# warmshao/ChatTTSPlus

Hardware: AMD Instinct MI355X
Metric: decode tokens/s (higher is better)
Workload: dtype f32

## Files before the change

### chatttsplus_amd/csrc/persist_layer.hip

```cpp
#include "kernels.h"
#include "persist.h"

typedef unsigned long long u64;

#ifndef PL_LB
#define PL_LB PL_THREADS_MAX
#endif
#define PL_SPIN_LIMIT (1u << 18)

typedef __attribute__((address_space(3))) int pl_lds_int;
#define PL_ABORT_GET(p_) __hip_atomic_load((pl_lds_int*)(p_), __ATOMIC_RELAXED, __HIP_MEMORY_SCOPE_WORKGROUP)
#define PL_ABORT_SET(p_) __hip_atomic_store((pl_lds_int*)(p_), 1, __ATOMIC_RELAXED, __HIP_MEMORY_SCOPE_WORKGROUP)
__device__ inline void store_granule(u64* g, unsigned tag, float v) {
    __hip_atomic_store(g, ((u64)tag << 32) | (u64)__builtin_bit_cast(unsigned, v), __ATOMIC_RELAXED, __HIP_MEMORY_SCOPE_AGENT);
}

template <int N, typename OffFn>
__device__ inline bool sweep(const u64* base, unsigned lane_elem, OffFn off, unsigned tag, float (&v)[N], int* err, int code, int* abort_s, int nap = 1) {
    const u64* p = base + lane_elem;
    asm volatile("" : "+v"(p));
#pragma unroll 1
    for (unsigned spins = 0;; ++spins) {
        bool ok = true;
#pragma unroll
// ... 705 lines not shown
                }
                if (last) PL_MARK(3);
                for (int z = 0; z < a.delay_att; ++z) __builtin_amdgcn_s_sleep(2);
                {
                    if (EW == 2 && (a.poll & 1)) watch_sentinels(a.g_att, [ew](int i) { return (i / 6) * PL_H + 64 * (2 * (i % 6) + ew) + 63; }, 6 * R, tag, lane, abort_s);
                    float v[GX * R];
                    const bool got = PL_SWEEP(GX * R, a.g_att, PL_G_ATT, (unsigned)e, [](int k) { return (k / GX) * PL_H + NE * (k % GX); }, tag, v, 3);
                    (void)got;
#pragma unroll
                    for (int k = 0; k < GX * R; ++k) xs[(k / GX) * PL_H + NE * (k % GX) + e] = v[k];
                }
                if (last) PL_MARK(4);
                PL_B1();
                float ldo = 0.f;
                float uo[LORA ? 16 : 1];
                const int slO = (LORA && e < 4 * R) ? pl_slot(a.lslots, e >> 2) : -1;
                if constexpr (LORA) {
                    for (int z = 0; z < a.delay_u; ++z) __builtin_amdgcn_s_sleep(2);
                    const bool got = sweep_masked<16>(a.g_u, (unsigned)((e >> 2) * 64 + 48), slO >= 0, tag, uo, a.error, 10, abort_s, a.nap);
                    (void)got;
                }
                __syncthreads();
                if constexpr (LORA) {
                    if (slO >= 0) {
                        const float* const bo = lbs + 192 * R + (e >> 2) * 64 + (e & 3) * 16;
#pragma unroll
                        for (int k = 0; k < 16; ++k) ldo = fmaf(bo[k], uo[k], ldo);
                    }
                }
                if (e < 4 * R) {
                    const int i = e & 3, r = e >> 2;
                    const float x1 = xres[4 * r + i] + (pl_red(red, i, r) + ldo);
                    xres[4 * r + i] = x1;
                    if (!(a.fault > 0 && b == 5 && l + 1 == a.fault))
                        store_granule(a.g_x1 + (size_t)pl_opq<(R > PL_MAXR_ONE)>(r * PL_H + 4 * b + i), tag, x1);
                }
                if (last) PL_MARK(5);
                for (int z = 0; z < a.delay; ++z) __builtin_amdgcn_s_sleep(2);
                {
                    if (EW == 2 && (a.poll & 1)) watch_sentinels(a.g_x1, [ew](int i) { return (R - 1) * PL_H + 4 * (16 * (2 * (i >> 4) + ew) + (i & 15)) + 3; }, 96, tag, lane, abort_s);
                    float v[GX * R];
                    const bool got = PL_SWEEP(GX * R, a.g_x1, PL_G_X1, (unsigned)e, [](int k) { return (k / GX) * PL_H + NE * (k % GX); }, tag, v, 4);
                    (void)got;
#pragma unroll
                    for (int r = 0; r < R; ++r) ssp[r] = 0.f;
#pragma unroll
                    for (int k = 0; k < GX * R; ++k) {
                        xs[(k / GX) * PL_H + NE * (k % GX) + e] = v[k];
                        ssp[k / GX] += v[k] * v[k];
                    }
#pragma unroll
                    for (int r = 0; r < R; ++r) {
                        const float s = wave_sum(ssp[r]);
                        if (lane == 0) ssq[ew * R + r] = s;
                    }
                }
                if (last) PL_MARK(6);
                PL_B1();
                __syncthreads();
                if constexpr (A16) {
                    float av = 0.f;
                    const int pi = e & 15, r = e >> 4;
                    if (e < 16 * R) {
                        const int w = pi >> 1, p = pi & 1;
                        const float rs = 1.0f / sqrtf((EW == 2 ? ssq[r] + ssq[R + r] : (ssq[r] + ssq[R + r]) + (ssq[2 * R + r] + ssq[3 * R + r])) / (float)PL_H + a.eps);
                        const float gv = pl_red(red, w, 16 * p + r) * rs, uv = pl_red(red, w, 16 * p + R + r) * rs;
                        av = (gv / (1.0f + expf(-gv))) * uv;
                    }
                    const float a1 = __shfl_down(av, 1), a2 = __shfl_down(av, 2);
                    if (e < 16 * R && pi % 3 == 0)
                        store_granule16(a.g_act, PL_GEMV_BLOCKS * PL_A16_SLOTS * R, (unsigned)pl_opq<(R > PL_MAXR_ONE)>((r * PL_GEMV_BLOCKS + b) * PL_A16_SLOTS + pi / 3), tag,
                                        av, (pi + 1 < 16) ? a1 : 0.f, (pi + 2 < 16) ? a2 : 0.f);
                } else if (e < 16 * R) {
                    const int pi = e & 15, r = e >> 4, w = pi >> 1, p = pi & 1;
                    const float rs = 1.0f / sqrtf((EW == 2 ? ssq[r] + ssq[R + r] : (ssq[r] + ssq[R + r]) + (ssq[2 * R + r] + ssq[3 * R + r])) / (float)PL_H + a.eps);
                    const float gv = pl_red(red, w, 16 * p + r) * rs, uv = pl_red(red, w, 16 * p + R + r) * rs;
                    store_granule(a.g_act + (size_t)pl_opq<(R > PL_MAXR_ONE)>(r * PL_I + 16 * b + pi), tag, (gv / (1.0f + expf(-gv))) * uv);
                }
                if (last) PL_MARK(7);
                for (int z = 0; z < a.delay_act; ++z) __builtin_amdgcn_s_sleep(2);
                if constexpr (A16) {
                    constexpr int TOT = PL_GEMV_BLOCKS * PL_A16_SLOTS * R, NK = (TOT + NE - 1) / NE;
                    constexpr int NC = (NK + PL_A16_CHUNK - 1) / PL_A16_CHUNK, CH = (NK + NC - 1) / NC;
                    act16_chunk<0, (NK < CH ? NK : CH), NE, TOT>(a.g_act, e, tag, (__attribute__((address_space(3))) float*)xs, a.error, abort_s, a.nap);
                    if constexpr (NC > 1) act16_chunk<CH, (NK - CH < CH ? NK - CH : CH), NE, TOT>(a.g_act, e, tag, (__attribute__((address_space(3))) float*)xs, a.error, abort_s, a.nap);
                    if constexpr (NC > 2) act16_chunk<2 * CH, (NK - 2 * CH < CH ? NK - 2 * CH : CH), NE, TOT>(a.g_act, e, tag, (__attribute__((address_space(3))) float*)xs, a.error, abort_s, a.nap);
                    if constexpr (NC > 3) act16_chunk<3 * CH, (NK - 3 * CH < CH ? NK - 3 * CH : CH), NE, TOT>(a.g_act, e, tag, (__attribute__((address_space(3))) float*)xs, a.error, abort_s, a.nap);
                    if constexpr (NC > 4) act16_chunk<4 * CH, NK - 4 * CH, NE, TOT>(a.g_act, e, tag, (__attribute__((address_space(3))) float*)xs, a.error, abort_s, a.nap);
                    static_assert(NC <= 5, "act gather: more chunks");
                } else {
                if (EW == 2 && (a.poll & 1)) watch_sentinels(a.g_act, [ew](int i) { return (R - 1) * PL_I + 16 * (8 * (i >> 2) + 4 * ew + (i & 3)) + 15; }, 96, tag, lane, abort_s);
                if constexpr (EW == 2) {
#pragma unroll
                    for (int r = 0; r < R; ++r) {
                        float v[24];
                        const bool got = sweep<24>(a.g_act, (unsigned)(r * PL_I + e), [](int k) { return 128 * k; }, tag, v, a.error, 5, abort_s, a.nap);
                        (void)got;
#pragma unroll
                        for (int k = 0; k < 24; ++k) xs[r * PL_I + 128 * k + e] = v[k];
                    }
                } else {
#ifdef PL_EXP_E1
                    if constexpr (R > PL_MAXR_ONE) {
#pragma unroll
                        for (int r = 0; r < R; ++r) {
                            float v[12];
                            const bool got = PL_SWEEP(12, a.g_act, PL_G_ACT, (unsigned)(r * PL_I + e), [](int k) { return 256 * k; }, tag, v, 5);
                            (void)got;
#pragma unroll
                            for (int k = 0; k < 12; ++k) xs[r * PL_I + 256 * k + e] = v[k];
                        }
                    } else
#endif
#pragma unroll
                    for (int r = 0; r + 1 < R; r += 2) {
                        float v[24];
                        const bool got = PL_SWEEP(24, a.g_act, PL_G_ACT, (unsigned)(r * PL_I + e), [](int k) { return (k / 12) * PL_I + 256 * (k % 12); }, tag, v, 5);
                        (void)got;
#pragma unroll
                        for (int k = 0; k < 24; ++k) xs[(r + k / 12) * PL_I + 256 * (k % 12) + e] = v[k];
                    }
#ifdef PL_EXP_E1
                    if constexpr ((R & 1) != 0 && R <= PL_MAXR_ONE) {
#else
                    if constexpr ((R & 1) != 0) {
#endif
                        constexpr int r = R - 1;
                        float v[12];
                        const bool got = PL_SWEEP(12, a.g_act, PL_G_ACT, (unsigned)(r * PL_I + e), [](int k) { return 256 * k; }, tag, v, 5);
                        (void)got;
#pragma unroll
                        for (int k = 0; k < 12; ++k) xs[r * PL_I + 256 * k + e] = v[k];
                    }
                }
                }
                if (last) PL_MARK(8);
                PL_B1();
                __syncthreads();
                if (e < 4 * R) {
                    const int i = e & 3, r = e >> 2;
                    const float x2 = xres[4 * r + i] + (pl_red(red, 2 * i, r) + pl_red(red, 2 * i + 1, r));
                    if (last && !a.heads) a.x[(size_t)r * PL_H + 4 * b + i] = x2;
                    else {
                        xres[4 * r + i] = x2;
                        store_granule(a.g_x + (size_t)pl_opq<(R > PL_MAXR_ONE)>(r * PL_H + 4 * b + i), tag, x2);
                    }
                }
            }
            if (a.heads) {
                const unsigned tagh = tag0 + (unsigned)(NL - 1);
                int4 hst = make_int4(1, 0, 0, 0);
                int hout = 0;
                float lnf_v = 0.f;
                if (e < 4 * R) {
                    hst = *(const int4*)(a.rows + (e >> 2));
                    hout = a.rows[e >> 2].out;
                    lnf_v = a.lnf[4 * b + (e & 3)];
                }
                for (int z = 0; z < a.delay_x; ++z) __builtin_amdgcn_s_sleep(2);
                float v[GX * R];
                const bool got = PL_SWEEP(GX * R, a.g_x, PL_G_X, (unsigned)e, [](int k) { return (k / GX) * PL_H + NE * (k % GX); }, tagh, v, 1);
                (void)got;
#pragma unroll
                for (int r = 0; r < R; ++r) ssp[r] = 0.f;
#pragma unroll
                for (int k = 0; k < GX * R; ++k) {
                    xs[(k / GX) * PL_H + NE * (k % GX) + e] = v[k];
                    ssp[k / GX] += v[k] * v[k];
                }
#pragma unroll
                for (int r = 0; r < R; ++r) {
                    const float s = wave_sum(ssp[r]);
                    if (lane == 0) ssq[ew * R + r] = s;
                }
                PL_B1();
                __syncthreads();
                if (e < PL_HEAD_ROWS * R) {
                    const int rr = e % PL_HEAD_ROWS, r = e / PL_HEAD_ROWS, col = PL_HEAD_ROWS * b + rr;
                    const float rs = 1.0f / sqrtf((EW == 2 ? ssq[r] + ssq[R + r] : (ssq[r] + ssq[R + r]) + (ssq[2 * R + r] + ssq[3 * R + r])) / (float)PL_H + a.eps);
                    if (col < a.n_valid) a.logits[(size_t)r * a.n_valid + col] = pl_red(red, rr >> 1, (rr & 1) * R + r) * rs;
                }
                if (e < 4 * R) {
                    float* const hid_out = ((SamplerDynPtr)a.dyn)->hidden_out;
                    if (hid_out != nullptr && hst.x == 0) {
                        const int i = e & 3, r = e >> 2;
                        const float rs = 1.0f / sqrtf((EW == 2 ? ssq[r] + ssq[R + r] : (ssq[r] + ssq[R + r]) + (ssq[2 * R + r] + ssq[3 * R + r])) / (float)PL_H + a.eps);
                        hid_out[(size_t)hout * ((SamplerDynPtr)a.dyn)->hidden_stride + (size_t)hst.y * PL_H + 4 * b + i] = lnf_v * (xres[4 * r + i] * rs);
                    }
                }
            }
            PL_MARK(9);
            if (a.ts != nullptr && e == 0) {
#pragma unroll
                for (int i = 0; i < 10; ++i) a.ts[(size_t)b * 10 + i] = t_mark[i];
            }
            if (b == 0 && e == 0) __hip_atomic_fetch_add(a.epoch, 1u, __ATOMIC_RELAXED, __HIP_MEMORY_SCOPE_AGENT);
        }
        return;
    }

    constexpr bool PAIR = R > PL_MAXR_ONE;
    constexpr int NWI = PAIR ? 4 : 8;
    const int S = PAIR ? 1 : a.S;
    const int isub = PAIR ? ((wave < 8) ? (wave >> 2) : ((wave - 8) & 1)) : 0;
    const int iw = PAIR ? (wave & 3) : wave;
    const int item = PAIR ? 2 * (b - PL_GEMV_BLOCKS) + isub : b - PL_GEMV_BLOCKS;
    if ((PAIR ? 2 * (b - PL_GEMV_BLOCKS) : item) >= PL_NH * R * S) return;
    const int rh = item / S, sp = item - rh * S;
    const int r = rh / PL_NH, hh = rh % PL_NH;
    float* const qs = att_s + 64 * isub;
    float* const ks = att_s + 128 + 64 * isub;
    float* const vs = att_s + 256 + 64 * isub;
    float* const mo = att_s + 384;
    float* const mm = mo + 512;
    float* const ml = mm + 8;
    const size_t kv_per = a.kv_per;
    if (wave < 8) {
        const RowMeta m = a.meta[r];
        const int kvc = (m.slot - m.kv_start + S - 1) / S;
        const int kv0 = m.kv_start + sp * kvc, kv1 = min(kv0 + kvc, m.slot);
        const int grp = lane >> 3, sub = lane & 7;
        const size_t head_base = ((size_t)m.seq * PL_NH + hh) * a.Lmax * CTTS_HEAD_DIM;
        constexpr int PRE = 6;
        constexpr int NT = (PAIR || PL_TAIL_ALL) ? PL_TAIL_IT : 0, PT = PRE + NT;
        constexpr int TB = sizeof(WT) == 4 ? 4096 : 2048;
        typedef __attribute__((address_space(3))) char lds_c;
        typedef __attribute__((address_space(1))) const void* gptr_t;
        lds_c* const tl = (lds_c*)smem + PL_FRONT_BYTES + wave * (NT * TB);
        PlKV<WT> kf[PRE];
        typename KvElem<WT>::reg vv[PRE][8];
        bool ok[PT];
        bool any_ok[PT];
#pragma unroll
        for (int u = 0; u < PT; ++u) {
            const int p = kv0 + 8 * (iw + NWI * u) + grp;
            ok[u] = p < kv1;
            any_ok[u] = kv0 + 8 * (iw + NWI * u) < kv1;
        }
#define PL_LOAD_KV(l_) do { const WT* const kb_ = (const WT*)a.kv + (size_t)(l_) * 2 * kv_per + head_base; const WT* const vb_ = kb_ + kv_per + lane; \
        _Pragma("unroll") for (int u = 0; u < PRE; ++u) if (any_ok[u]) { const int p0_ = kv0 + 8 * (iw + NWI * u); const int pc_ = ok[u] ? p0_ + grp : m.kv_start; \
            kf[u].load(kb_ + (size_t)pc_ * CTTS_HEAD_DIM + 8 * sub); \
            _Pragma("unroll") for (int g = 0; g < 8; ++g) vv[u][g] = KvElem<WT>::load(vb_ + (size_t)min(p0_ + g, kv1 - 1) * CTTS_HEAD_DIM); } } while (0)
#define PL_DMA_KV(l_) do { if constexpr (NT > 0) { const WT* const kb_ = (const WT*)a.kv + (size_t)(l_) * 2 * kv_per + head_base; const WT* const vb_ = kb_ + kv_per; \
        int ln_ = lane; asm volatile("" : "+v"(ln_));       \
        const int grp = ln_ >> 3, sub = ln_ & 7, lane = ln_; \
        _Pragma("unroll") for (int t = 0; t < NT; ++t) if (any_ok[PRE + t]) { const int p0_ = kv0 + 8 * (iw + NWI * (PRE + t)); \
            const WT* const ks_ = kb_ + (size_t)min(p0_ + grp, kv1 - 1) * CTTS_HEAD_DIM + 8 * sub; \
            if constexpr (sizeof(WT) == 4) { \
                __builtin_amdgcn_global_load_lds((gptr_t)ks_, (__attribute__((address_space(3))) void*)(tl + t * TB), 16, 0, 0); \
                __builtin_amdgcn_global_load_lds((gptr_t)(ks_ + 4), (__attribute__((address_space(3))) void*)(tl + t * TB + 1024), 16, 0, 0); \
                const WT* const v0_ = vb_ + (size_t)min(p0_ + (lane >> 4), kv1 - 1) * CTTS_HEAD_DIM + 4 * (lane & 15); \
                const WT* const v1_ = vb_ + (size_t)min(p0_ + 4 + (lane >> 4), kv1 - 1) * CTTS_HEAD_DIM + 4 * (lane & 15); \
                __builtin_amdgcn_global_load_lds((gptr_t)v0_, (__attribute__((address_space(3))) void*)(tl + t * TB + 2048), 16, 0, 0); \
                __builtin_amdgcn_global_load_lds((gptr_t)v1_, (__attribute__((address_space(3))) void*)(tl + t * TB + 3072), 16, 0, 0); \
            } else { \
                __builtin_amdgcn_global_load_lds((gptr_t)ks_, (__attribute__((address_space(3))) void*)(tl + t * TB), 16, 0, 0); \
                const WT* const v0_ = vb_ + (size_t)min(p0_ + grp, kv1 - 1) * CTTS_HEAD_DIM + 8 * sub; \
                __builtin_amdgcn_global_load_lds((gptr_t)v0_, (__attribute__((address_space(3))) void*)(tl + t * TB + 1024), 16, 0, 0); \
            } } } } while (0)
        PL_DMA_KV(0);
        PL_LOAD_KV(0);
        __builtin_amdgcn_sched_barrier(0);
        if (__builtin_amdgcn_readfirstlane(done_v | err_v)) return;
        __syncthreads();
        for (int l = 0; l < NL; ++l) {
            const WT* const kb = (const WT*)a.kv + (size_t)l * 2 * kv_per + head_base + 8 * sub;
            const WT* const vb = (const WT*)a.kv + (size_t)l * 2 * kv_per + kv_per + head_base + lane;
            __syncthreads();
#define PL_AMARK(i) do { if (a.ts != nullptr && l + 1 == NL && tid == 0) a.ts[(size_t)b * 10 + (i)] = wall_clock64(); } while (0)
            PL_AMARK(3);
            const f32x4 q0 = *(const f32x4*)(qs + 8 * sub), q1 = *(const f32x4*)(qs + 8 * sub + 4);
            float sc[PT];
            float mw = -INFINITY;
#pragma unroll
            for (int u = 0; u < PRE; ++u) {
                sc[u] = -INFINITY;
                if (any_ok[u]) {
                    float dot = q0[0] * kf[u].at(0) + q0[1] * kf[u].at(1) + q0[2] * kf[u].at(2) + q0[3] * kf[u].at(3) +
                                q1[0] * kf[u].at(4) + q1[1] * kf[u].at(5) + q1[2] * kf[u].at(6) + q1[3] * kf[u].at(7);
                    dot += dpp_f<DPP_XOR1>(dot);
                    dot += dpp_f<DPP_XOR2>(dot);
                    dot += dpp_f<DPP_HALF_MIRROR>(dot);
                    sc[u] = ok[u] ? dot : -INFINITY;
                    mw = fmaxf(mw, sc[u]);
                }
            }
            if constexpr (NT > 0) {
                asm volatile("s_waitcnt vmcnt(0)" ::: "memory");
#pragma unroll
                for (int t = 0; t < NT; ++t) {
                    sc[PRE + t] = -INFINITY;
                    if (any_ok[PRE + t]) {
                        PlKV<WT> kt;
                        if constexpr (sizeof(WT) == 4) { kt.a = *(const __attribute__((address_space(3))) f32x4*)(tl + t * TB + lane * 16); kt.b = *(const __attribute__((address_space(3))) f32x4*)(tl + t * TB + 1024 + lane * 16); }
                        else kt.h = *(const __attribute__((address_space(3))) half8*)(tl + t * TB + lane * 16);
                        float dot = q0[0] * kt.at(0) + q0[1] * kt.at(1) + q0[2] * kt.at(2) + q0[3] * kt.at(3) + q1[0] * kt.at(4) + q1[1] * kt.at(5) + q1[2] * kt.at(6) + q1[3] * kt.at(7);
                        dot += dpp_f<DPP_XOR1>(dot);
                        dot += dpp_f<DPP_XOR2>(dot);
                        dot += dpp_f<DPP_HALF_MIRROR>(dot);
                        sc[PRE + t] = ok[PRE + t] ? dot : -INFINITY;
                        mw = fmaxf(mw, sc[PRE + t]);
                    }
                }
            }
            float mrun = wave_max(mw);
            PL_AMARK(4);
            float lrun = 0.f;
            float oa[4] = {0.f, 0.f, 0.f, 0.f};
#pragma unroll
            for (int u = 0; u < PRE; ++u) {
                if (any_ok[u]) {
                    const float pe = (sc[u] == -INFINITY) ? 0.f : expf(sc[u] - mrun);
                    lrun += pe;
#pragma unroll
                    for (int g = 0; g < 8; ++g) oa[g & 3] = fmaf(readlane_f(pe, 8 * g), KvElem<WT>::f(vv[u][g]), oa[g & 3]);
                }
            }
            if constexpr (NT > 0) {
#pragma unroll
                for (int t = 0; t < NT; ++t) {
                    if (any_ok[PRE + t]) {
                        const float pe = (sc[PRE + t] == -INFINITY) ? 0.f : expf(sc[PRE + t] - mrun);
                        lrun += pe;
#pragma unroll
                        for (int g = 0; g < 8; ++g) {
                            float vt;
                            if constexpr (sizeof(WT) == 4) vt = *(const __attribute__((address_space(3))) float*)(tl + t * TB + 2048 + g * 256 + lane * 4);
                            else vt = (float)*(const __attribute__((address_space(3))) half_t*)(tl + t * TB + 1024 + g * 128 + lane * 2);
                            oa[g & 3] = fmaf(readlane_f(pe, 8 * g), vt, oa[g & 3]);
                        }
                    }
                }
            }
            constexpr int UNS = 4, STEP = 8 * NWI;
            for (int wb0 = kv0 + 8 * (iw + NWI * PT); wb0 < kv1; wb0 += STEP * UNS) {
                PlKV<WT> ks_[UNS];
                typename KvElem<WT>::reg vs_[UNS][8];
                bool live_[UNS];
#pragma unroll
                for (int u = 0; u < UNS; ++u) {
// ... 250 lines not shown
```

### chatttsplus_amd/csrc/sampler.hip

```cpp
#include "kernels.h"

#define VPL 10

__device__ inline uint4 philox4x32_10(uint4 c, uint2 k) {
#pragma unroll
    for (int r = 0; r < 10; ++r) {
        const unsigned hi0 = __umulhi(0xD2511F53u, c.x), lo0 = 0xD2511F53u * c.x;
        const unsigned hi1 = __umulhi(0xCD9E8D57u, c.z), lo1 = 0xCD9E8D57u * c.z;
        c = make_uint4(hi1 ^ c.y ^ k.x, lo1, hi0 ^ c.w ^ k.y, lo0);
        k.x += 0x9E3779B9u; k.y += 0xBB67AE85u;
    }
    return c;
}

struct RowIn {
    const float* q;
    int myid;
    float T;
    bool penalize;
    int step;
    unsigned long long seed;
    unsigned uid_lo, uid_hi;
    unsigned vq, attempt;
};
// ... 59 lines not shown
    float myv = -INFINITY;
    int myi = 0, nsel = 0;
    unsigned kept = 0;
    bool fast = false;
    if (topk <= 64) {
        unsigned vkey[VPL], head = 0u;
#pragma unroll
        for (int i = 0; i < VPL; ++i) { vkey[i] = ((valid >> i) & 1u) ? f32_key(x[i]) : 0u; head = max(head, vkey[i]); }
        int greater = 0;
#pragma unroll
        for (int j = 0; j < 64; ++j) greater += ((unsigned)__builtin_amdgcn_readlane((int)head, j) > head) ? 1 : 0;
        const unsigned long long t0k = wave_max_u64((greater < topk) ? (unsigned long long)(~head) : 0ull);
        const unsigned T0 = ~(unsigned)t0k;
        int C = 0;
        int pos[VPL];
#pragma unroll
        for (int i = 0; i < VPL; ++i) {
            const bool cand = ((valid >> i) & 1u) && vkey[i] >= T0;
            const unsigned long long bal = __builtin_amdgcn_ballot_w64(cand);
            pos[i] = cand ? C + (int)__builtin_amdgcn_mbcnt_hi((unsigned)(bal >> 32), __builtin_amdgcn_mbcnt_lo((unsigned)bal, 0u)) : -1;
            C += __builtin_popcountll(bal);
        }
        if (C <= 64) {
            fast = true;
#pragma unroll
            for (int i = 0; i < VPL; ++i)
                if (pos[i] >= 0) lds64[pos[i]] = ((unsigned long long)vkey[i] << 32) | (unsigned)(lane + 64 * i);
            __builtin_amdgcn_fence(__ATOMIC_RELEASE, "wavefront");
            __builtin_amdgcn_wave_barrier();
            __builtin_amdgcn_fence(__ATOMIC_ACQUIRE, "wavefront");
            const unsigned long long ck = (lane < C) ? lds64[lane] : 0ull;
            int rank = 0;
            for (int j = 0; j < C; ++j) rank += (readlane_u64(ck, j) > ck) ? 1 : 0;
            const unsigned lo = (unsigned)__builtin_amdgcn_ds_permute(rank << 2, (int)(unsigned)ck);
            const unsigned hi = (unsigned)__builtin_amdgcn_ds_permute(rank << 2, (int)(unsigned)(ck >> 32));
            const float bv = key_f32(hi);
            const int bi = (int)lo;
            const float p_r = (lane < C) ? expf(bv - mx) * inv : 0.f;
            const float vk = readlane_f(bv, (topk - 1) & 63);
            double cum = 0.0, cum_mine = 0.0;
            for (int r = 0; r < C; ++r) {
                if (lane == r) cum_mine = cum;
                cum += (double)readlane_f(p_r, r);
            }
            const float cr = (float)(tot - cum_mine);
            const bool stop = (lane >= C) || (lane >= topk && bv != vk) || (cr <= c.top_p_threshold && lane >= c.min_keep);
            const unsigned long long sb = __builtin_amdgcn_ballot_w64(stop);
            nsel = (sb == 0ull) ? 64 : (int)__builtin_ctzll(sb);
            myv = bv; myi = bi;
        }
    }
    if (!fast) {
        unsigned long long key[VPL];
#pragma unroll
        for (int i = 0; i < VPL; ++i)
            key[i] = ((valid >> i) & 1u) ? (((unsigned long long)f32_key(x[i]) << 32) | (unsigned)(lane + 64 * i)) : 0ull;
#pragma unroll
        for (int pass = 0; pass < VPL; ++pass)
#pragma unroll
            for (int i = pass & 1; i + 1 < VPL; i += 2) {
                const unsigned long long a = key[i], b = key[i + 1];
                key[i] = a > b ? a : b;
                key[i + 1] = a > b ? b : a;
            }
        double cum_before = 0.0;
        float vk = 0.f;
        for (int r = 0; r < V; ++r) {
            const unsigned long long best = wave_max_u64(key[0]);
            if (best == 0ull) break;
            const float bv = key_f32((unsigned)(best >> 32));
            const int bi = (int)(unsigned)best;
            const int owner = bi & 63, slot = bi >> 6;
            if (r >= topk && bv != vk) break;
            const float cr = (float)(tot - cum_before);
            if (cr <= c.top_p_threshold && r >= c.min_keep) break;
            if (lane == owner) {
                kept |= 1u << slot;
#pragma unroll
                for (int i = 0; i + 1 < VPL; ++i) key[i] = key[i + 1];
                key[VPL - 1] = 0ull;
            }
            if (lane == r) { myv = bv; myi = bi; }
            nsel = r + 1;
            if (r == topk - 1) vk = bv;
            cum_before += (double)(expf(bv - mx) * inv);
        }
        if (in.step < c.min_new) {
            if (lane == (c.eos & 63)) kept &= ~(1u << (c.eos >> 6));
        }
    }
    unsigned long long bkey = 0ull;
    if (nsel <= 64) {
        const bool on = (lane < nsel) && !(in.step < c.min_new && myi == c.eos);
        const float m2 = wave_max(on ? myv : -INFINITY);
        const float e = on ? expf(myv - m2) : 0.f;
        const float inv2 = 1.0f / wave_sum(e);
        bkey = ((unsigned long long)f32_key(0.f) << 32) | (unsigned)0x7FFFFFFF;
        if (on) {
            const float ratio = __fdiv_rn(e * inv2, exp_noise_of(in, myi));
            bkey = umax64(bkey, ((unsigned long long)f32_key(ratio) << 32) | (unsigned)(0x7FFFFFFF - myi));
        }
        bkey = wave_max_u64(bkey);
        if (want_lp) {
            const bool mine = on && myi == 0x7FFFFFFF - (int)(unsigned)bkey;
            lp_sampled = wave_max(mine ? logf(e * inv2) : -INFINITY);
        }
    } else {
        float m2 = -INFINITY;
#pragma unroll
        for (int i = 0; i < VPL; ++i) if ((kept >> i) & 1u) m2 = fmaxf(m2, x[i]);
        m2 = wave_max(m2);
        float e2[VPL], s2 = 0.f;
#pragma unroll
        for (int i = 0; i < VPL; ++i) { e2[i] = ((kept >> i) & 1u) ? expf(x[i] - m2) : 0.f; s2 += e2[i]; }
        s2 = wave_sum(s2);
        const float inv2 = 1.0f / s2;
#pragma unroll
        for (int i = 0; i < VPL; ++i) {
            const int j = lane + 64 * i;
            if (j < V) {
                float ratio = 0.f;
                if ((kept >> i) & 1u) ratio = __fdiv_rn(e2[i] * inv2, exp_noise_of(in, j));
                bkey = umax64(bkey, ((unsigned long long)f32_key(ratio) << 32) | (unsigned)(0x7FFFFFFF - j));
            }
        }
        bkey = wave_max_u64(bkey);
        if (want_lp) {
            const int bi = 0x7FFFFFFF - (int)(unsigned)bkey;
            float pe = 0.f;
#pragma unroll
            for (int i = 0; i < VPL; ++i) pe = (i == (bi >> 6)) ? e2[i] : pe;
            lp_sampled = readlane_f(logf(pe * inv2), bi & 63);
        }
    }
    const int besti = 0x7FFFFFFF - (int)(unsigned)bkey;
    if (want_lp) {
        float rm = -INFINITY;
#pragma unroll
        for (int i = 0; i < VPL; ++i) rm = ((valid >> i) & 1u) ? fmaxf(rm, lg[i]) : rm;
        rm = wave_max(rm);
        float rs = 0.f, rv = 0.f;
#pragma unroll
        for (int i = 0; i < VPL; ++i) {
            const float t = lg[i] - rm;
            rs += ((valid >> i) & 1u) ? expf(t) : 0.f;
            rv = (i == (besti >> 6)) ? t : rv;
        }
        rs = wave_sum(rs);
        lp_raw = readlane_f(rv, besti & 63) - logf(rs);
    }
    return besti;
}

__global__ __launch_bounds__(256) void sampler_generate_kernel(const int* st_words, const float* logits_p, const SamplerDyn* dyn_p, const RowMeta* meta_p,
                                                               const int V_p, const int* ring_p, const RowState* finend_p, const SamplerArgs a) {
    __shared__ float tab[17];
    __shared__ int idx_s[CTTS_NUM_VQ];
    __shared__ unsigned long long cand_s[CTTS_NUM_VQ][64];
    DevState* st = a.st;
    const SamplerDynPtr d = (SamplerDynPtr)dyn_p;
    const int tid = threadIdx.x, lane = tid & 63, vq = tid >> 6;
    const int b = blockIdx.x;
    int zoff;
    asm volatile("v_mov_b32 %0, 0" : "=v"(zoff));
    const int4 hdr = *(const int4*)(st_words + zoff);
    float lg[VPL];
    {
        const float* lrow = logits_p + (size_t)(b * CTTS_NUM_VQ + vq) * V_p;
#pragma unroll
        for (int i = 0; i < VPL; ++i) { const int j = lane + 64 * i; lg[i] = (j < V_p) ? lrow[j] : 0.f; }
    }
    const int ring_v = ring_p[(size_t)(b * CTTS_NUM_VQ + vq) * 16 + (lane & 15)];
    const int4 fe = ((const int4*)(finend_p + b))[0];
    const int4 uid = ((const int4*)(finend_p + b))[1];
    const CTTS_CONST_AS RowSampling* knob = (const CTTS_CONST_AS RowSampling*)(finend_p + CTTS_MAX_B) + b;
    if (tid < 17) tab[tid] = knob->penalty_table[tid];
    const RowMeta meta_in = meta_p[b];
    if (__builtin_amdgcn_readfirstlane(hdr.z)) return;
    const int gstep = __builtin_amdgcn_readfirstlane(hdr.x), draw = __builtin_amdgcn_readfirstlane(hdr.y);
    const int fin_in = fe.x, end_in = fe.y;
    const int step = end_in;
    const int seq = uid.z;
    const float rope_next = (tid < 64) ? a.rope[(size_t)(meta_in.pos + 1) * 64 + tid] : 0.f;
    __syncthreads();
    const int row = seq * CTTS_NUM_VQ + vq;
    RowIn in;
    in.q = (d->noise != nullptr) ? d->noise + ((size_t)min(draw, d->n_draws - 1) * d->rows0 + row) * a.V : nullptr;
    const int nh = min(step, knob->past_window);
    const int age = ((step - 1 - lane) & 15) + 1;
    in.myid = (lane < 16 && age <= nh) ? ring_v : -1;
    in.T = knob->temperature[vq];
    in.penalize = knob->use_penalty && (b * CTTS_NUM_VQ + vq < d->cfg.max_input_ids) && nh > 0;
    in.step = step;
    in.seed = d->seed; in.uid_lo = (unsigned)uid.x; in.uid_hi = (unsigned)uid.y; in.vq = (unsigned)vq; in.attempt = (unsigned)fe.z;
    SampleKnobs kn;
    kn.top_p_threshold = knob->top_p_threshold; kn.top_k = knob->top_k; kn.min_keep = knob->min_keep; kn.eos = d->cfg.eos; kn.min_new = knob->min_new;
    float* const lp_raw_out = d->lp_raw;
    float* const lp_smp_out = d->lp_sampled;
    const bool want_lp = (lp_raw_out != nullptr) || (lp_smp_out != nullptr);
    float lp_raw = 0.f, lp_smp = 0.f;
    const int idx = sample_row(kn, tab, in, a.V, lane, lg, cand_s[vq], want_lp, lp_raw, lp_smp);
    if (lane == 0) {
        idx_s[vq] = idx;
        if (fin_in == 0) {
            const size_t at = ((size_t)seq * d->cfg.max_new + step) * CTTS_NUM_VQ + vq;
            d->ids[at] = idx;
            if (lp_raw_out != nullptr) lp_raw_out[at] = lp_raw;
            if (lp_smp_out != nullptr) lp_smp_out[at] = lp_smp;
        }
        a.hist_ring[(size_t)(b * CTTS_NUM_VQ + vq) * 16 + (step & 15)] = idx;
    }
    __syncthreads();
    for (int k = tid; k < a.H; k += 256) {
        float s = a.emb_code[((size_t)0 * a.V + idx_s[0]) * a.H + k];
#pragma unroll
        for (int v = 1; v < CTTS_NUM_VQ; ++v) s += a.emb_code[((size_t)v * a.V + idx_s[v]) * a.H + k];
        a.x_next[(size_t)b * a.H + k] = s;
    }
    if (tid == 0) {
        const bool was = fin_in != 0;
        bool eos = (fin_in & 2) != 0;
        for (int v = 0; v < CTTS_NUM_VQ; ++v) eos = eos || (idx_s[v] == d->cfg.eos);
        bool fin = was || eos;
        const int end_out = fin ? end_in : end_in + 1;
        if (!fin) d->end_idx[seq] = end_out;
        fin = fin || (end_out >= fe.w);
        if (!was) d->finish[seq] = eos ? 1 : 0;
        ((int2*)(a.finend + b))[0] = make_int2(fin ? (eos ? 3 : 1) : 0, end_out);
        if (!was) {
            RowMeta m = meta_in;
            m.pos += 1; m.slot += 1;
            a.meta[b] = m;
        }
        const int add = 1 + ((fin && !was) ? 0x10000 : 0);
        const int tot = (a.B == 1) ? (__builtin_amdgcn_readfirstlane(hdr.w) + add) : (__hip_atomic_fetch_add(&st->ticket, add, __ATOMIC_RELAXED, __HIP_MEMORY_SCOPE_AGENT) + add);
        if ((tot & 0xFFFF) == a.B) {
            const int nfin = tot >> 16;
            st->ticket = nfin << 16;
            st->step = gstep + 1;
            st->draw = draw + 1;
            if (nfin == a.B) st->all_done = 1;
        }
    }
    if (tid < 64) a.rope_rows[(size_t)b * 64 + tid] = rope_next;
}

#define TVPT 21
struct BlockRed {
    float f[16];
    double d[16];
    unsigned long long k[16];
    unsigned long long k2[2][16];
};
__device__ inline float block_max_f(BlockRed& r, float v, int lane, int wave) {
    v = wave_max(v);
    if (lane == 0) r.f[wave] = v;
    __syncthreads();
    float m = r.f[0];
#pragma unroll
    for (int i = 1; i < 16; ++i) m = fmaxf(m, r.f[i]);
    __syncthreads();
    return m;
}
__device__ inline float block_sum_f(BlockRed& r, float v, int lane, int wave) {
    v = wave_sum(v);
    if (lane == 0) r.f[wave] = v;
    __syncthreads();
    float m = 0.f;
#pragma unroll
    for (int i = 0; i < 16; ++i) m += r.f[i];
    __syncthreads();
    return m;
}
__device__ inline double block_sum_d(BlockRed& r, double v, int lane, int wave) {
    v = wave_sum_d(v);
    if (lane == 0) r.d[wave] = v;
    __syncthreads();
    double m = 0.0;
#pragma unroll
    for (int i = 0; i < 16; ++i) m += r.d[i];
    __syncthreads();
    return m;
}
__device__ inline unsigned long long block_max_u64(BlockRed& r, unsigned long long v, int lane, int wave) {
    v = wave_max_u64(v);
    if (lane == 0) r.k[wave] = v;
    __syncthreads();
    unsigned long long m = r.k[0];
#pragma unroll
    for (int i = 1; i < 16; ++i) m = umax64(m, r.k[i]);
    __syncthreads();
    return m;
}

__device__ inline unsigned long long block_max_u64_alt(BlockRed& r, unsigned long long v, int lane, int wave, int round) {
    v = wave_max_u64(v);
    unsigned long long* slot = r.k2[round & 1];
    if (lane == 0) slot[wave] = v;
    __syncthreads();
    unsigned long long m = slot[0];
#pragma unroll
    for (int i = 1; i < 16; ++i) m = umax64(m, slot[i]);
    return m;
}

__global__ __launch_bounds__(1024) void sampler_text_kernel(const SamplerArgs a) {
    __shared__ BlockRed red;
    __shared__ int pos_s;
    DevState* st = a.st;
    const SamplerDynPtr d = (SamplerDynPtr)a.dyn;
    if (st->all_done) return;
    const int tid = threadIdx.x, lane = tid & 63, wave = tid >> 6;
    const int b = blockIdx.x, V = a.V;
    const int gstep = st->step, draw = st->draw;
    const RowState rs_in = a.finend[b];
    const int step = rs_in.end, seq = rs_in.out;
    const float* lg = a.logits + (size_t)b * V;
    const float* q = (d->noise != nullptr) ? d->noise + ((size_t)min(draw, d->n_draws - 1) * d->rows0 + seq) * V : nullptr;
    const float T = d->cfg.temperature[0];
    float x[TVPT];
    unsigned valid = 0;
#pragma unroll
    for (int i = 0; i < TVPT; ++i) {
        const int j = tid + 1024 * i;
        if (j < V) { x[i] = __fdiv_rn(lg[j], T); valid |= 1u << i; }
        else x[i] = -INFINITY;
    }
    float mx = -INFINITY;
#pragma unroll
    for (int i = 0; i < TVPT; ++i) mx = fmaxf(mx, x[i]);
    mx = block_max_f(red, mx, lane, wave);
    float se = 0.f;
#pragma unroll
    for (int i = 0; i < TVPT; ++i) se += ((valid >> i) & 1u) ? expf(x[i] - mx) : 0.f;
    se = block_sum_f(red, se, lane, wave);
    const float inv = 1.0f / se;
    double tot = 0.0;
#pragma unroll
    for (int i = 0; i < TVPT; ++i) tot += ((valid >> i) & 1u) ? (double)(expf(x[i] - mx) * inv) : 0.0;
    tot = block_sum_d(red, tot, lane, wave);

    unsigned taken = ~valid, kept = 0;
    const int topk = (d->cfg.top_k > 0) ? d->cfg.top_k : V;
    __shared__ unsigned top2_s[16][2];
    __shared__ int wtot_s[16];
    __shared__ unsigned long long cand_s[64];
    __shared__ int sel_s[64];
    __shared__ int nsel_s;
    bool fast = false;
    if (topk <= 32) {
        unsigned vkey[TVPT], head = 0u;
#pragma unroll
        for (int i = 0; i < TVPT; ++i) { vkey[i] = ((valid >> i) & 1u) ? f32_key(x[i]) : 0u; head = max(head, vkey[i]); }
        const unsigned long long hk = ((unsigned long long)head << 32) | (unsigned)lane;
        const unsigned long long b1 = wave_max_u64(hk);
        const unsigned long long b2 = wave_max_u64(hk == b1 ? 0ull : hk);
        if (lane == 0) { top2_s[wave][0] = (unsigned)(b1 >> 32); top2_s[wave][1] = (unsigned)(b2 >> 32); }
        __syncthreads();
        const unsigned mine32 = (lane < 32) ? top2_s[lane >> 1][lane & 1] : 0u;
        int greater = 0;
#pragma unroll
        for (int j = 0; j < 32; ++j) greater += (top2_s[j >> 1][j & 1] > mine32) ? 1 : 0;
        const unsigned T0 = ~(unsigned)wave_max_u64((lane < 32 && greater < topk) ? (unsigned long long)(~mine32) : 0ull);
        unsigned cmask = 0;
#pragma unroll
        for (int i = 0; i < TVPT; ++i) cmask |= (((valid >> i) & 1u) && vkey[i] >= T0) ? (1u << i) : 0u;
        const int cnt = __builtin_popcount(cmask);
        int incl = cnt;
#pragma unroll
        for (int off = 1; off < 64; off <<= 1) { const int t = __shfl_up(incl, off); if (lane >= off) incl += t; }
        if (lane == 63) wtot_s[wave] = incl;
        __syncthreads();
        int base = 0, C = 0;
#pragma unroll
        for (int w = 0; w < 16; ++w) { base += (w < wave) ? wtot_s[w] : 0; C += wtot_s[w]; }
        if (C <= 64) {
            fast = true;
            int pos = base + incl - cnt;
#pragma unroll
            for (int i = 0; i < TVPT; ++i)
                if ((cmask >> i) & 1u) cand_s[pos++] = ((unsigned long long)vkey[i] << 32) | (unsigned)(tid + 1024 * i);
            __syncthreads();
            if (wave == 0) {
                const unsigned long long ck = (lane < C) ? cand_s[lane] : 0ull;
                int rank = 0;
                for (int j = 0; j < C; ++j) rank += (readlane_u64(ck, j) > ck) ? 1 : 0;
                const unsigned lo = (unsigned)__builtin_amdgcn_ds_permute(rank << 2, (int)(unsigned)ck);
                const unsigned hi = (unsigned)__builtin_amdgcn_ds_permute(rank << 2, (int)(unsigned)(ck >> 32));
                const float bv = key_f32(hi);
                const float p_r = (lane < C) ? expf(bv - mx) * inv : 0.f;
                const float vk = readlane_f(bv, (topk - 1) & 63);
                double cum = 0.0, cum_mine = 0.0;
                for (int r = 0; r < C; ++r) {
                    if (lane == r) cum_mine = cum;
                    cum += (double)readlane_f(p_r, r);
                }
                const float cr = (float)(tot - cum_mine);
// ... 349 lines not shown
```

Before: 3903.

## Batch sampler parameter loads into per-lane dwords and overlap embedding gather with bookkeeping

The sampler kernel now loads the RowSampling and SamplerDyn structs as one dword per lane up front and pulls fields out with readlane. This replaces the scattered scalar or constant loads that sat on the critical path. It also issues all logits and state loads before the first use, gives each wave its own penalty table with only a wave barrier, and for H=768 starts the embedding gather before the bookkeeping writes. The persistent layer's head path similarly prefetches the hidden_out pointer and stride before the sweep, which adds code complexity and relies on the exact struct layout.

```diff
diff --git a/chatttsplus_amd/csrc/persist_layer.hip b/chatttsplus_amd/csrc/persist_layer.hip
--- a/chatttsplus_amd/csrc/persist_layer.hip
+++ b/chatttsplus_amd/csrc/persist_layer.hip
@@ -881,11 +881,21 @@
                 int4 hst = make_int4(1, 0, 0, 0);
                 int hout = 0;
                 float lnf_v = 0.f;
+                int2 hid_w = make_int2(0, 0);
+                int hid_stride = 0;
                 if (e < 4 * R) {
                     hst = *(const int4*)(a.rows + (e >> 2));
                     hout = a.rows[e >> 2].out;
                     lnf_v = a.lnf[4 * b + (e & 3)];
-                }
+                    int z;
+                    asm volatile("v_mov_b32 %0, 0" : "=v"(z));
+                    const int* const dynw = (const int*)a.dyn + z;
+                    hid_w = *(const int2*)(dynw + offsetof(SamplerDyn, hidden_out) / 4);
+                    hid_stride = dynw[offsetof(SamplerDyn, hidden_stride) / 4];
+                }
+                float* const logits_out = a.logits;
+                const int n_valid = a.n_valid;
+                asm volatile("" : : "s"(logits_out), "s"(n_valid));
                 for (int z = 0; z < a.delay_x; ++z) __builtin_amdgcn_s_sleep(2);
                 float v[GX * R];
                 const bool got = PL_SWEEP(GX * R, a.g_x, PL_G_X, (unsigned)e, [](int k) { return (k / GX) * PL_H + NE * (k % GX); }, tagh, v, 1);
@@ -907,14 +917,15 @@
                 if (e < PL_HEAD_ROWS * R) {
                     const int rr = e % PL_HEAD_ROWS, r = e / PL_HEAD_ROWS, col = PL_HEAD_ROWS * b + rr;
                     const float rs = 1.0f / sqrtf((EW == 2 ? ssq[r] + ssq[R + r] : (ssq[r] + ssq[R + r]) + (ssq[2 * R + r] + ssq[3 * R + r])) / (float)PL_H + a.eps);
-                    if (col < a.n_valid) a.logits[(size_t)r * a.n_valid + col] = pl_red(red, rr >> 1, (rr & 1) * R + r) * rs;
+                    if (col < n_valid) logits_out[(size_t)r * n_valid + col] = pl_red(red, rr >> 1, (rr & 1) * R + r) * rs;
                 }
                 if (e < 4 * R) {
-                    float* const hid_out = ((SamplerDynPtr)a.dyn)->hidden_out;
+                    float __attribute__((address_space(1)))* const hid_out =
+                        (float __attribute__((address_space(1)))*)((unsigned long long)(unsigned)hid_w.x | ((unsigned long long)(unsigned)hid_w.y << 32));
                     if (hid_out != nullptr && hst.x == 0) {
                         const int i = e & 3, r = e >> 2;
                         const float rs = 1.0f / sqrtf((EW == 2 ? ssq[r] + ssq[R + r] : (ssq[r] + ssq[R + r]) + (ssq[2 * R + r] + ssq[3 * R + r])) / (float)PL_H + a.eps);
-                        hid_out[(size_t)hout * ((SamplerDynPtr)a.dyn)->hidden_stride + (size_t)hst.y * PL_H + 4 * b + i] = lnf_v * (xres[4 * r + i] * rs);
+                        hid_out[(size_t)hout * hid_stride + (size_t)hst.y * PL_H + 4 * b + i] = lnf_v * (xres[4 * r + i] * rs);
                     }
                 }
             }
diff --git a/chatttsplus_amd/csrc/sampler.hip b/chatttsplus_amd/csrc/sampler.hip
--- a/chatttsplus_amd/csrc/sampler.hip
+++ b/chatttsplus_amd/csrc/sampler.hip
@@ -235,97 +235,155 @@
     return besti;
 }
 
+#define KNOB_WORD(field) ((int)(offsetof(RowSampling, field) / 4))
+#define DYN_WORD(field) ((int)(offsetof(SamplerDyn, field) / 4))
+static_assert(sizeof(RowSampling) / 4 <= 64 && sizeof(SamplerDyn) / 4 <= 64, "one dword per lane");
+static_assert(sizeof(SamplerDyn) % 4 == 0 && offsetof(SamplerDyn, ids) % 8 == 0, "SamplerDyn is read as dwords");
+#define ARRIVE_V(x) asm volatile("" : "+v"(x))
+#define ARRIVE_S(x) asm volatile("" : : "s"(x))
+__device__ inline int lane_word(int v, int w) { return __builtin_amdgcn_readlane(v, w); }
+#define CTTS_GLOBAL_AS __attribute__((address_space(1)))
+template <typename T> __device__ inline CTTS_GLOBAL_AS T* lane_ptr(int v, int w) {
+    const unsigned long long lo = (unsigned)__builtin_amdgcn_readlane(v, w), hi = (unsigned)__builtin_amdgcn_readlane(v, w + 1);
+    return (CTTS_GLOBAL_AS T*)(lo | (hi << 32));
+}
+
 __global__ __launch_bounds__(256) void sampler_generate_kernel(const int* st_words, const float* logits_p, const SamplerDyn* dyn_p, const RowMeta* meta_p,
                                                                const int V_p, const int* ring_p, const RowState* finend_p, const SamplerArgs a) {
-    __shared__ float tab[17];
+    __shared__ float tab[CTTS_NUM_VQ][20];
     __shared__ int idx_s[CTTS_NUM_VQ];
     __shared__ unsigned long long cand_s[CTTS_NUM_VQ][64];
-    DevState* st = a.st;
-    const SamplerDynPtr d = (SamplerDynPtr)dyn_p;
-    const int tid = threadIdx.x, lane = tid & 63, vq = tid >> 6;
+    const int tid = threadIdx.x, lane = tid & 63, vq = __builtin_amdgcn_readfirstlane(tid >> 6);
     const int b = blockIdx.x;
     int zoff;
     asm volatile("v_mov_b32 %0, 0" : "=v"(zoff));
-    const int4 hdr = *(const int4*)(st_words + zoff);
+    int4 hdr = *(const int4*)(st_words + zoff);
     float lg[VPL];
     {
         const float* lrow = logits_p + (size_t)(b * CTTS_NUM_VQ + vq) * V_p;
 #pragma unroll
-        for (int i = 0; i < VPL; ++i) { const int j = lane + 64 * i; lg[i] = (j < V_p) ? lrow[j] : 0.f; }
-    }
-    const int ring_v = ring_p[(size_t)(b * CTTS_NUM_VQ + vq) * 16 + (lane & 15)];
-    const int4 fe = ((const int4*)(finend_p + b))[0];
-    const int4 uid = ((const int4*)(finend_p + b))[1];
-    const CTTS_CONST_AS RowSampling* knob = (const CTTS_CONST_AS RowSampling*)(finend_p + CTTS_MAX_B) + b;
-    if (tid < 17) tab[tid] = knob->penalty_table[tid];
-    const RowMeta meta_in = meta_p[b];
+        for (int i = 0; i < VPL; ++i) lg[i] = lrow[min(lane + 64 * i, V_p - 1)];
+    }
+    int ring_v = ring_p[(size_t)(b * CTTS_NUM_VQ + vq) * 16 + (lane & 15)];
+    int4 fe = ((const int4*)(finend_p + b))[0];
+    int4 uid = ((const int4*)(finend_p + b))[1];
+    int kw = ((const int*)((const RowSampling*)(finend_p + CTTS_MAX_B) + b))[min(lane, (int)(sizeof(RowSampling) / 4) - 1)];
+    int dw = ((const int*)dyn_p)[min(lane, (int)(sizeof(SamplerDyn) / 4) - 1)];
+    int4 meta_w = *(const int4*)(meta_p + b);
+    __builtin_amdgcn_sched_barrier(0);
+    const float* const emb_code = a.emb_code;
+    const float* const rope = a.rope;
+    float* const x_next = a.x_next;
+    float* const rope_rows = a.rope_rows;
+    const int H = a.H, B = a.B;
+    ARRIVE_S(emb_code); ARRIVE_S(rope); ARRIVE_S(x_next); ARRIVE_S(rope_rows); ARRIVE_S(H); ARRIVE_S(B);
+    ARRIVE_V(hdr.x); ARRIVE_V(ring_v); ARRIVE_V(fe.x); ARRIVE_V(uid.x); ARRIVE_V(kw); ARRIVE_V(dw); ARRIVE_V(meta_w.x);
+#pragma unroll
+    for (int i = 0; i < VPL; ++i) ARRIVE_V(lg[i]);
+    __builtin_amdgcn_sched_barrier(0);
     if (__builtin_amdgcn_readfirstlane(hdr.z)) return;
+    const int V = V_p;
+#pragma unroll
+    for (int i = 0; i < VPL; ++i) lg[i] = (lane + 64 * i < V) ? lg[i] : 0.f;
     const int gstep = __builtin_amdgcn_readfirstlane(hdr.x), draw = __builtin_amdgcn_readfirstlane(hdr.y);
-    const int fin_in = fe.x, end_in = fe.y;
+    const int fin_in = __builtin_amdgcn_readfirstlane(fe.x), end_in = __builtin_amdgcn_readfirstlane(fe.y);
+    const int attempt = __builtin_amdgcn_readfirstlane(fe.z), limit = __builtin_amdgcn_readfirstlane(fe.w);
     const int step = end_in;
-    const int seq = uid.z;
-    const float rope_next = (tid < 64) ? a.rope[(size_t)(meta_in.pos + 1) * 64 + tid] : 0.f;
-    __syncthreads();
+    const int seq = __builtin_amdgcn_readfirstlane(uid.z);
+    const int pos = __builtin_amdgcn_readfirstlane(meta_w.y);
+    const float rope_next = (tid < 64) ? rope[(size_t)(pos + 1) * 64 + tid] : 0.f;
+    if (lane >= KNOB_WORD(penalty_table) && lane < KNOB_WORD(penalty_table) + 17) tab[vq][lane - KNOB_WORD(penalty_table)] = __builtin_bit_cast(float, kw);
+    __builtin_amdgcn_fence(__ATOMIC_RELEASE, "wavefront");
+    __builtin_amdgcn_wave_barrier();
+    __builtin_amdgcn_fence(__ATOMIC_ACQUIRE, "wavefront");
+    CTTS_GLOBAL_AS const float* const noise = lane_ptr<const float>(dw, DYN_WORD(noise));
+    CTTS_GLOBAL_AS int* const ids_out = lane_ptr<int>(dw, DYN_WORD(ids));
+    CTTS_GLOBAL_AS int* const finish_out = lane_ptr<int>(dw, DYN_WORD(finish));
+    CTTS_GLOBAL_AS int* const end_idx_out = lane_ptr<int>(dw, DYN_WORD(end_idx));
+    CTTS_GLOBAL_AS float* const lp_raw_out = lane_ptr<float>(dw, DYN_WORD(lp_raw));
+    CTTS_GLOBAL_AS float* const lp_smp_out = lane_ptr<float>(dw, DYN_WORD(lp_sampled));
+    const int n_draws = lane_word(dw, DYN_WORD(n_draws)), rows0 = lane_word(dw, DYN_WORD(rows0));
+    const int eos = lane_word(dw, DYN_WORD(cfg.eos)), max_new = lane_word(dw, DYN_WORD(cfg.max_new)), max_input_ids = lane_word(dw, DYN_WORD(cfg.max_input_ids));
     const int row = seq * CTTS_NUM_VQ + vq;
     RowIn in;
-    in.q = (d->noise != nullptr) ? d->noise + ((size_t)min(draw, d->n_draws - 1) * d->rows0 + row) * a.V : nullptr;
-    const int nh = min(step, knob->past_window);
+    in.q = (noise != nullptr) ? (const float*)(noise + ((size_t)min(draw, n_draws - 1) * rows0 + row) * V) : nullptr;
+    const int nh = min(step, lane_word(kw, KNOB_WORD(past_window)));
     const int age = ((step - 1 - lane) & 15) + 1;
     in.myid = (lane < 16 && age <= nh) ? ring_v : -1;
-    in.T = knob->temperature[vq];
-    in.penalize = knob->use_penalty && (b * CTTS_NUM_VQ + vq < d->cfg.max_input_ids) && nh > 0;
+    in.T = __builtin_bit_cast(float, __builtin_amdgcn_readlane(kw, KNOB_WORD(temperature) + vq));
+    in.penalize = lane_word(kw, KNOB_WORD(use_penalty)) && (b * CTTS_NUM_VQ + vq < max_input_ids) && nh > 0;
     in.step = step;
-    in.seed = d->seed; in.uid_lo = (unsigned)uid.x; in.uid_hi = (unsigned)uid.y; in.vq = (unsigned)vq; in.attempt = (unsigned)fe.z;
+    in.seed = ((unsigned long long)(unsigned)lane_word(dw, DYN_WORD(seed) + 1) << 32) | (unsigned)lane_word(dw, DYN_WORD(seed));
+    in.uid_lo = (unsigned)__builtin_amdgcn_readfirstlane(uid.x); in.uid_hi = (unsigned)__builtin_amdgcn_readfirstlane(uid.y);
+    in.vq = (unsigned)vq; in.attempt = (unsigned)attempt;
     SampleKnobs kn;
-    kn.top_p_threshold = knob->top_p_threshold; kn.top_k = knob->top_k; kn.min_keep = knob->min_keep; kn.eos = d->cfg.eos; kn.min_new = knob->min_new;
-    float* const lp_raw_out = d->lp_raw;
-    float* const lp_smp_out = d->lp_sampled;
+    kn.top_p_threshold = __builtin_bit_cast(float, lane_word(kw, KNOB_WORD(top_p_threshold)));
+    kn.top_k = lane_word(kw, KNOB_WORD(top_k)); kn.min_keep = lane_word(kw, KNOB_WORD(min_keep)); kn.eos = eos; kn.min_new = lane_word(kw, KNOB_WORD(min_new));
     const bool want_lp = (lp_raw_out != nullptr) || (lp_smp_out != nullptr);
     float lp_raw = 0.f, lp_smp = 0.f;
-    const int idx = sample_row(kn, tab, in, a.V, lane, lg, cand_s[vq], want_lp, lp_raw, lp_smp);
+    const int idx = sample_row(kn, tab[vq], in, V, lane, lg, cand_s[vq], want_lp, lp_raw, lp_smp);
     if (lane == 0) {
         idx_s[vq] = idx;
         if (fin_in == 0) {
-            const size_t at = ((size_t)seq * d->cfg.max_new + step) * CTTS_NUM_VQ + vq;
-            d->ids[at] = idx;
+            const size_t at = ((size_t)seq * max_new + step) * CTTS_NUM_VQ + vq;
+            ids_out[at] = idx;
             if (lp_raw_out != nullptr) lp_raw_out[at] = lp_raw;
             if (lp_smp_out != nullptr) lp_smp_out[at] = lp_smp;
         }
-        a.hist_ring[(size_t)(b * CTTS_NUM_VQ + vq) * 16 + (step & 15)] = idx;
-    }
-    __syncthreads();
-    for (int k = tid; k < a.H; k += 256) {
-        float s = a.emb_code[((size_t)0 * a.V + idx_s[0]) * a.H + k];
-#pragma unroll
-        for (int v = 1; v < CTTS_NUM_VQ; ++v) s += a.emb_code[((size_t)v * a.V + idx_s[v]) * a.H + k];
-        a.x_next[(size_t)b * a.H + k] = s;
-    }
-    if (tid == 0) {
+        const_cast<int*>(ring_p)[(size_t)(b * CTTS_NUM_VQ + vq) * 16 + (step & 15)] = idx;
+    }
+    __syncthreads();
+    int id4[CTTS_NUM_VQ];
+#pragma unroll
+    for (int v = 0; v < CTTS_NUM_VQ; ++v) id4[v] = __builtin_amdgcn_readfirstlane(idx_s[v]);
+    auto bookkeeping = [&]() {
+        if (tid != 0) return;
         const bool was = fin_in != 0;
-        bool eos = (fin_in & 2) != 0;
-        for (int v = 0; v < CTTS_NUM_VQ; ++v) eos = eos || (idx_s[v] == d->cfg.eos);
-        bool fin = was || eos;
+        bool eos_seen = (fin_in & 2) != 0;
+        for (int v = 0; v < CTTS_NUM_VQ; ++v) eos_seen = eos_seen || (id4[v] == eos);
+        bool fin = was || eos_seen;
         const int end_out = fin ? end_in : end_in + 1;
-        if (!fin) d->end_idx[seq] = end_out;
-        fin = fin || (end_out >= fe.w);
-        if (!was) d->finish[seq] = eos ? 1 : 0;
-        ((int2*)(a.finend + b))[0] = make_int2(fin ? (eos ? 3 : 1) : 0, end_out);
+        if (!fin) end_idx_out[seq] = end_out;
+        fin = fin || (end_out >= limit);
+        if (!was) finish_out[seq] = eos_seen ? 1 : 0;
+        ((int2*)const_cast<RowState*>(finend_p + b))[0] = make_int2(fin ? (eos_seen ? 3 : 1) : 0, end_out);
         if (!was) {
-            RowMeta m = meta_in;
-            m.pos += 1; m.slot += 1;
-            a.meta[b] = m;
-        }
+            int4 m = meta_w;
+            m.y += 1; m.z += 1;
+            *(int4*)const_cast<RowMeta*>(meta_p + b) = m;
+        }
+        DevState* st = (DevState*)const_cast<int*>(st_words);
         const int add = 1 + ((fin && !was) ? 0x10000 : 0);
-        const int tot = (a.B == 1) ? (__builtin_amdgcn_readfirstlane(hdr.w) + add) : (__hip_atomic_fetch_add(&st->ticket, add, __ATOMIC_RELAXED, __HIP_MEMORY_SCOPE_AGENT) + add);
-        if ((tot & 0xFFFF) == a.B) {
+        const int tot = (B == 1) ? (__builtin_amdgcn_readfirstlane(hdr.w) + add) : (__hip_atomic_fetch_add(&st->ticket, add, __ATOMIC_RELAXED, __HIP_MEMORY_SCOPE_AGENT) + add);
+        if ((tot & 0xFFFF) == B) {
             const int nfin = tot >> 16;
             st->ticket = nfin << 16;
             st->step = gstep + 1;
             st->draw = draw + 1;
-            if (nfin == a.B) st->all_done = 1;
-        }
-    }
-    if (tid < 64) a.rope_rows[(size_t)b * 64 + tid] = rope_next;
+            if (nfin == B) st->all_done = 1;
+        }
+    };
+    if (H == 768) {
+        float e[3][CTTS_NUM_VQ];
+#pragma unroll
+        for (int c = 0; c < 3; ++c)
+#pragma unroll
+            for (int v = 0; v < CTTS_NUM_VQ; ++v) e[c][v] = emb_code[((size_t)v * V + id4[v]) * 768 + tid + 256 * c];
+        __builtin_amdgcn_sched_barrier(0);
+        bookkeeping();
+        __builtin_amdgcn_sched_barrier(0);
+#pragma unroll
+        for (int c = 0; c < 3; ++c) x_next[(size_t)b * 768 + tid + 256 * c] = ((e[c][0] + e[c][1]) + e[c][2]) + e[c][3];
+    } else {
+        bookkeeping();
+        for (int k = tid; k < H; k += 256) {
+            float s = emb_code[((size_t)0 * V + id4[0]) * H + k];
+#pragma unroll
+            for (int v = 1; v < CTTS_NUM_VQ; ++v) s += emb_code[((size_t)v * V + id4[v]) * H + k];
+            x_next[(size_t)b * H + k] = s;
+        }
+    }
+    if (tid < 64) rope_rows[(size_t)b * 64 + tid] = rope_next;
 }
 
 #define TVPT 21
```

Result: faster. 3960 (median of 6 runs) (+1.5%).
